# ten2net/Gym-Trading-Env

Hardware: AMD Instinct MI355X
Metric: env-steps/sec (higher is better)
Workload: dtype f64

## Files before the change

gym-trading-env_amd/csrc/gte_api.hip:

```cpp
#include <hip/hip_runtime.h>

#include <climits>
#include <cstdarg>
#include <cstdio>
#include <cstdlib>
#include <cstring>
#include <new>
#include <string>
#include <utility>
#include <vector>

#include "gte_launch.h"
#include "gte_ledger.h"
#include "gte_plan.h"

using gte::DatasetDesc;
using gte::EnvRec;
using gte::Params;
using gte_plan::LaunchPlan;
using gte_plan::SLIDE_AB_ORDER;
using gte_ledger::FLAGS;
using gte_ledger::WINDOW;
using gte_ledger::ledger;

// ... 380 lines not shown
  }
  double* d_pos = nullptr;
  chk(dev_alloc(E, &d_pos, GTE_MAX_POSITIONS));
  chk(dev_alloc(E, &E->d_ds, (size_t)p.D));
  if (rc == GTE_OK &&
      hipMemcpy(d_pos, cfg->positions, sizeof(double) * p.P, hipMemcpyHostToDevice) != hipSuccess)
    rc = fail(GTE_ERR_HIP, "copying positions failed");
  if (rc != GTE_OK) return create_failed(E, rc);
  p.positions = d_pos;
  p.ds = E->d_ds;
  E->owned.obs_elems_per_env = (int64_t)p.W * p.Fobs;
  p.final_obs = nullptr;
  p.obs = nullptr; p.reward = E->owned.reward; p.reward64 = E->owned.reward64;
  p.obs_rows = p.W; p.obs_head = 0; p.slide = 0;
  p.terminated = E->owned.terminated; p.truncated = E->owned.truncated;
  E->term_base = E->owned.term_count; p.term_ids = E->owned.term_ids;
  E->h_ds.assign((size_t)p.D, DatasetDesc{nullptr, nullptr, nullptr, nullptr, 0});
  for (auto& v : E->ds_allocs) v.assign((size_t)p.D, nullptr);

  rc = plan_launches(E);
  if (rc != GTE_OK) return create_failed(E, rc);
  if (hipDeviceSynchronize() != hipSuccess)
    return create_failed(E, fail(GTE_ERR_HIP, "hipDeviceSynchronize failed after allocation"));
  report_plan(E, "create");
  *out = E;
  return GTE_OK;
}

static int publish_signal_table(gte_env* E, int32_t d, const gte::SignalTable& t) {
  const gte::SignalTable before = E->h_sig[d];
  E->h_sig[d] = t;
  const hipError_t e = hipMemcpy(E->d_sig, E->h_sig.data(), sizeof(gte::SignalTable) * E->h_sig.size(),
                                 hipMemcpyHostToDevice);
  if (e != hipSuccess) {
    E->h_sig[d] = before;
    return fail(GTE_ERR_HIP, "publishing the signal table of dataset %d: %s", d, hipGetErrorString(e));
  }
  bool any = false;
  for (const gte::SignalTable& x : E->h_sig) any = any || x.base != nullptr;
  if (!any) E->sig_S = 0;
  return GTE_OK;
}

static int publish_period_row(gte_env* E, int32_t d, const gte::PeriodRow& r) {
  const gte::PeriodRow before = E->h_prow[d];
  E->h_prow[d] = r;
  const hipError_t e = hipMemcpy(E->d_prow, E->h_prow.data(), sizeof(gte::PeriodRow) * E->h_prow.size(),
                                 hipMemcpyHostToDevice);
  if (e != hipSuccess) {
    E->h_prow[d] = before;
    return fail(GTE_ERR_HIP, "publishing the period row of dataset %d: %s", d, hipGetErrorString(e));
  }
  if (before.base) (void)hipFree(const_cast<int8_t*>(before.base));
  if (E->pd_B > 0) E->pd_changed = true;
  return GTE_OK;
}

int gte_upload_dataset(gte_env* E, int32_t d, const float* feat, const double* close,
                       const double* high, const double* low, int64_t T) {
  if (!E) return fail(GTE_ERR_INVALID, "env is NULL");
  const Params& p = E->p;
  if (d < 0 || d >= p.D) return fail(GTE_ERR_INVALID, "dataset index %d out of range", d);
  if (!feat || !close) return fail(GTE_ERR_INVALID, "feat and close are required");
  if (T <= 0 || T > 0x7FFFFFF0ll) return fail(GTE_ERR_INVALID, "T out of range");
  const int64_t idx0 = p.has_window ? p.W - 1 : 0;
  if (T < idx0 + 2) return fail(GTE_ERR_INVALID, "dataset of %lld rows is too short for windows=%d",
                                (long long)T, p.W);
  if (p.max_dur > 0 && T - p.max_dur - idx0 <= idx0)
    return fail(GTE_ERR_INVALID, "low >= high: %lld rows cannot host episodes of %d steps",
                (long long)T, p.max_dur);
  if (E->finalized && p.persist && T > p.depth)
    return fail(GTE_ERR_STATE, "dyn_persist: cannot upload a longer dataset after the first reset");
  if (E->was_reset && T < E->h_ds[d].T)
    return fail(GTE_ERR_STATE, "dataset %d: cannot replace %lld rows by %lld after gte_reset "
                "(running environments may be past the new end); create a new env instead",
                d, (long long)E->h_ds[d].T, (long long)T);
  HIPCHK(hipSetDevice(E->cfg.device));
  HIPCHK(hipStreamSynchronize(E->stream));
  const void* srcs[4] = {feat, close, high, low};
  const size_t bytes[4] = {sizeof(float) * (size_t)T * p.Fobs, sizeof(double) * (size_t)T,
                           sizeof(double) * (size_t)T, sizeof(double) * (size_t)T};
  void* dev[4] = {nullptr, nullptr, nullptr, nullptr};
  auto undo = [&]() { for (void* q : dev) if (q) (void)hipFree(q); };
  for (int k = 0; k < 4; ++k) {
    if (!srcs[k]) continue;
    hipError_t e = hipMalloc(&dev[k], bytes[k]);
    if (e == hipSuccess && getenv("GTE_DEBUG_ALLOC"))
      fprintf(stderr, "[gte] dataset %d column %d at %p, %zu bytes\n", d, k, dev[k], bytes[k]);
    if (e == hipSuccess) e = hipMemcpy(dev[k], srcs[k], bytes[k], hipMemcpyHostToDevice);
    if (e != hipSuccess) {
      undo();
      return fail(e == hipErrorOutOfMemory ? GTE_ERR_OOM : GTE_ERR_HIP, "uploading dataset %d: %s", d,
                  hipGetErrorString(e));
    }
  }
  const DatasetDesc before = E->h_ds[d];
  E->h_ds[d] = DatasetDesc{(const float*)dev[0], (const double*)dev[1], (const double*)dev[2],
                           (const double*)dev[3], T};
  const hipError_t e = hipMemcpy(E->d_ds, E->h_ds.data(), sizeof(DatasetDesc) * p.D, hipMemcpyHostToDevice);
  if (e != hipSuccess) {
    E->h_ds[d] = before;
    undo();
    return fail(GTE_ERR_HIP, "publishing the descriptor of dataset %d: %s", d, hipGetErrorString(e));
  }
  for (int k = 0; k < 4; ++k) {
    if (E->ds_allocs[k][d]) (void)hipFree(E->ds_allocs[k][d]);
    E->ds_allocs[k][d] = dev[k];
  }
  if (E->d_sig && E->h_sig[d].base) TRY(publish_signal_table(E, d, gte::SignalTable{nullptr, 0}));
  if (E->d_prow && E->h_prow[d].base) TRY(publish_period_row(E, d, gte::PeriodRow{nullptr, 0}));
  return GTE_OK;
}

static int finalize(gte_env* E) {
  if (E->finalized) return GTE_OK;
  Params& p = E->p;
  int64_t maxT = 0;
  for (int d = 0; d < p.D; ++d) {
    if (E->h_ds[d].T <= 0) return fail(GTE_ERR_STATE, "dataset %d was never uploaded", d);
    if (E->h_ds[d].T > maxT) maxT = E->h_ds[d].T;
  }
  p.depth = p.persist ? maxT : p.W;
  size_t table_bytes = 0;
  for (int d = 0; d < p.D; ++d) table_bytes += (size_t)E->h_ds[d].T * p.Fobs * sizeof(float);
  gte_plan::affinity_after_upload(E->plan, plan_shape(E), table_bytes);
  TRY(dev_alloc(E, &p.ring, (size_t)p.N * p.depth * (p.nd ? p.nd : 1)));
  HIPCHK(hipDeviceSynchronize());
  report_plan(E, "finalize");
  E->finalized = true;
  return GTE_OK;
}

static int check_injection(const gte_env* E, size_t count, const int32_t* idx, const int32_t* pos,
                           const int32_t* ds) {
  const Params& p = E->p;
  int64_t maxT = 0, minT = INT64_MAX;
  for (int d = 0; d < p.D; ++d) {
    if (E->h_ds[d].T > maxT) maxT = E->h_ds[d].T;
    if (E->h_ds[d].T > 0 && E->h_ds[d].T < minT) minT = E->h_ds[d].T;
  }
  const int64_t idx0 = p.has_window ? p.W - 1 : 0;
  for (size_t i = 0; i < count; ++i) {
    if (pos && pos[i] >= p.P) return fail(GTE_ERR_INVALID, "injected position index %d >= %d", pos[i], p.P);
    if (ds && ds[i] >= p.D) return fail(GTE_ERR_INVALID, "injected dataset %d >= %d", ds[i], p.D);
    if (idx && idx[i] >= 0) {
      const int64_t T = (ds && ds[i] >= 0) ? E->h_ds[ds[i]].T : minT;
      if (idx[i] < idx0 || idx[i] > T - 2)
        return fail(GTE_ERR_INVALID, "injected start row %d outside [%lld, %lld]", idx[i],
                    (long long)idx0, (long long)(T - 2));
    }
  }
  return GTE_OK;
}

static int append_log(gte_env* E, const Params& p, const uint8_t* mask = nullptr) {
  if (E->cfg.log_steps <= 0) return GTE_OK;
  if (E->log_rows == 0) mask = nullptr;
  HIPCHK(gte::launch_log(p.rec, p.reward64, p.terminated, p.truncated, p.N, E->log_cursor + (E->term_slot ^ 1),
                         E->cfg.log_steps, E->log, mask, E->stream));
  if (!mask) E->log_rows += 1;
  return GTE_OK;
}

static int park_cursor(gte_env* E, int slot) {
  if (!E->log_cursor || E->term_slot == slot) return GTE_OK;
  HIPCHK(hipMemcpyAsync(E->log_cursor + slot, E->log_cursor + E->term_slot, sizeof(int64_t),
                        hipMemcpyDeviceToDevice, E->stream));
  return GTE_OK;
}

static int stage(gte_env* E, void* dst, const void* src, size_t bytes) {
  HIPCHK(hipMemcpyAsync(dst, src, bytes, hipMemcpyHostToDevice, E->stream));
  return GTE_OK;
}

static int ensure_owned_obs(gte_env* E) {
  Params& p = E->p;
  const size_t elems = (size_t)p.N * (size_t)p.W * (size_t)p.Fobs;
  bool fresh = false;
  if (!p.obs) {
    if (!E->owned.obs) { TRY(dev_alloc(E, &E->owned.obs, elems)); fresh = true; }
    p.obs = E->owned.obs;
  }
  if (E->cfg.final_obs && !p.final_obs) {
    if (!E->owned.final_obs) { TRY(dev_alloc(E, &E->owned.final_obs, elems)); fresh = true; }
    p.final_obs = E->owned.final_obs;
  }
  if (fresh) HIPCHK(hipDeviceSynchronize());
  return GTE_OK;
}

static int resort(gte_env* E) {
  E->steps_since_rebuild = 0;
  const hipError_t e = gte::launch_affinity_rebuild(E->p, E->d_bins, E->plan.n_bins_per_ds,
                                                    E->d_slot_of_rank, E->d_perm, E->stream);
  if (e != hipSuccess) {
    E->plan.affinity_period = 0;
    E->p.perm = nullptr;
    return fail(GTE_ERR_HIP, "re-sort of the processing order: %s", hipGetErrorString(e));
  }
  E->p.perm = E->d_perm;
  return GTE_OK;
}

int gte_reset(gte_env* E, const uint8_t* mask, const int32_t* inj_idx,
              const int32_t* inj_pos_index, const int32_t* inj_dataset) {
  if (!E) return fail(GTE_ERR_INVALID, "env is NULL");
  HIPCHK(hipSetDevice(E->cfg.device));
  TRY(ensure_owned_obs(E));
  TRY(finalize(E));
  TRY(check_injection(E, (size_t)E->p.N, inj_idx, inj_pos_index, inj_dataset));
  Params p = E->p;
  const bool fresh_run = E->sliding && !mask;
  if (fresh_run) p.obs_head = 0;
  ledger().wrote(E, {obs_span(E), flag_span(E, p.terminated), flag_span(E, p.truncated)}, false,
                 fresh_run ? FLAGS | WINDOW : FLAGS);
  const size_t N = (size_t)p.N;
  p.mask = nullptr; p.inj_idx = p.inj_pos = p.inj_ds = nullptr;
  if (mask) { TRY(stage(E, E->d_mask, mask, N)); p.mask = E->d_mask; }
  if (inj_idx) { TRY(stage(E, E->d_inj_idx, inj_idx, 4 * N)); p.inj_idx = E->d_inj_idx; }
  if (inj_pos_index) { TRY(stage(E, E->d_inj_pos, inj_pos_index, 4 * N)); p.inj_pos = E->d_inj_pos; }
  if (inj_dataset) { TRY(stage(E, E->d_inj_ds, inj_dataset, 4 * N)); p.inj_ds = E->d_inj_ds; }
  HIPCHK(hipMemsetAsync(E->term_base, 0, 2 * sizeof(int32_t), E->stream));
  TRY(park_cursor(E, 1));
  E->term_slot = 0;
  p.term_count = E->term_base;
  p.term_count_next = E->term_base + 1;
  const LaunchPlan& L = E->plan;
  HIPCHK(gte::launch_reset(p, L.vec, L.store, L.coop, L.stage, L.blocks, L.threads, E->stream));
  if (fresh_run) {
    E->p.obs_head = 0;
    ledger().establish(E, WINDOW, {obs_span(E)}, false);
  }
  TRY(append_log(E, p, p.mask));
  if (L.affinity_period > 0) TRY(resort(E));
  HIPCHK(hipStreamSynchronize(E->stream));
  E->was_reset = true;
  return GTE_OK;
}

int gte_set_autoreset_injection(gte_env* E, int32_t n, const int32_t* inj_idx,
                                const int32_t* inj_pos_index, const int32_t* inj_dataset) {
  if (!E) return fail(GTE_ERR_INVALID, "env is NULL");
  if (n < 0) return fail(GTE_ERR_INVALID, "n_episodes must be >= 0");
  for (int d = 0; d < E->p.D; ++d)
    if (E->h_ds[d].T <= 0) return fail(GTE_ERR_STATE, "upload every dataset before queueing draws");
  TRY(check_injection(E, (size_t)E->p.N * (size_t)n, inj_idx, inj_pos_index, inj_dataset));
  HIPCHK(hipSetDevice(E->cfg.device));
  HIPCHK(hipStreamSynchronize(E->stream));
  Params& p = E->p;
  const size_t count = (size_t)p.N * (size_t)n;
  auto put = [&](int32_t** slot, const int32_t* src, const int32_t** param) -> int {
    *param = nullptr;
    if (*slot) { (void)hipFree(*slot); *slot = nullptr; }
    if (!src || n == 0) return GTE_OK;
    void* dev = nullptr;
    HIPCHK(hipMalloc(&dev, sizeof(int32_t) * count));
    *slot = (int32_t*)dev;
    HIPCHK(hipMemcpy(dev, src, sizeof(int32_t) * count, hipMemcpyHostToDevice));
    *param = *slot;
    return GTE_OK;
  };
  TRY(put(&E->d_q_idx, inj_idx, &p.q_idx));
  TRY(put(&E->d_q_pos, inj_pos_index, &p.q_pos));
  TRY(put(&E->d_q_ds, inj_dataset, &p.q_ds));
  p.q_n = n;
  HIPCHK(gte::launch_rewind_queue(p.rec, p.N, E->stream));
  HIPCHK(hipStreamSynchronize(E->stream));
  HIPCHK(hipDeviceSynchronize());
  return GTE_OK;
}

static bool stream_capturing(gte_env* E) {
  hipStreamCaptureStatus capture = hipStreamCaptureStatusNone;
  if (hipStreamIsCapturing(E->stream, &capture) != hipSuccess) { (void)hipGetLastError(); capture = hipStreamCaptureStatusNone; }
  return capture == hipStreamCaptureStatusActive;
}

static void advance_term_slot(gte_env* E, Params& p) {
  E->term_slot ^= 1;
  p.term_count = E->term_base + E->term_slot;
  p.term_count_next = E->term_base + (E->term_slot ^ 1);
}

struct StepTargets {
  const int32_t* actions;
  float *obs, *reward;
  double* reward64;
  uint8_t *terminated, *truncated;
  bool own_obs;
};

static StepTargets own_targets(const gte_env* E, const int32_t* actions) {
  return {actions, E->p.obs, E->p.reward, E->p.reward64, E->p.terminated, E->p.truncated, true};
}

static int age_order(gte_env* E, int32_t steps) {
  if (E->plan.affinity_period > 0 && (E->steps_since_rebuild += steps) >= E->plan.affinity_period) {
    TRY(resort(E));
  }
  return GTE_OK;
}

static int enqueue_step(gte_env* E, const StepTargets& t, int store, bool capturing,
                        EnvRec* terminal_rec = nullptr) {
  const LaunchPlan& L = E->plan;
  const bool slides_own = t.own_obs && E->sliding;
  gte_ledger::Span obs = obs_span(E);
  const bool slide = slides_own && !capturing && ledger().holds(E, WINDOW, {obs}) && E->p.obs_head < L.slide_rows;
  const bool env_order = slide && !L.full_windows && !(L.slide_ab & SLIDE_AB_ORDER);
  if (env_order) { if (L.affinity_period > 0) E->steps_since_rebuild += 1; }
  else TRY(age_order(E, 1));
  Params p = E->p;
  if (env_order) p.perm = nullptr;
  if (terminal_rec) p.final_rec = terminal_rec;
  p.actions = t.actions; p.obs = t.obs; p.reward = t.reward; p.reward64 = t.reward64;
  p.terminated = t.terminated; p.truncated = t.truncated;
  if (!t.own_obs) {
    p.obs_rows = p.W; p.obs_head = 0;
    obs = {t.obs, sizeof(float) * (size_t)p.N * p.W * p.Fobs};
  } else if (E->sliding) {
    if (slide) {
      E->p.obs_head += 1;
      if (p.persist || p.final_obs)
        return fail(GTE_ERR_STATE, "internal: a sliding step with dyn_persist or final_obs (the planner grants neither)");
      p.slide = L.full_windows ? 0 : 1;
    } else {
      E->p.obs_head = 0;
    }
    p.obs_head = E->p.obs_head;
  }
  advance_term_slot(E, p);
  if (L.fused_log) {
    p.log = E->log;
    p.log_cursor = E->log_cursor + (E->term_slot ^ 1);
  }
  const gte_ledger::Span term = flag_span(E, p.terminated), trunc = flag_span(E, p.truncated);
  p.flags_sparse = !capturing && !L.always_dense && ledger().holds(E, FLAGS, {term, trunc}) ? 1 : 0;
  ledger().wrote(E, {obs, term, trunc}, capturing, FLAGS | WINDOW);
  const bool hot = L.hot_tu && gte::hot_tu_covers(p);
  if (p.slide) store = L.slide_store;
  if (hot && store == 2)
    HIPCHK(gte::launch_step_hot(p, L.blocks, L.threads, gte::lds_bytes(p, L.stage), E->stream));
  else if (hot && store == 1)
    HIPCHK(gte::launch_step_hot_nt(p, L.blocks, L.threads, gte::lds_bytes(p, L.stage), E->stream));
  else
    HIPCHK(gte::launch_step(p, L.vec, store, L.coop, L.stage, L.blocks, L.threads, E->stream));
  ledger().establish(E, FLAGS, {term, trunc}, capturing);
  if (slides_own) ledger().establish(E, WINDOW, {obs}, capturing);
  if (L.fused_log) E->log_rows += 1;
  else TRY(append_log(E, p));
  return GTE_OK;
}

int gte_step(gte_env* E, const int32_t* actions, int32_t actions_on_device) {
  if (!E) return fail(GTE_ERR_INVALID, "env is NULL");
  if (!E->was_reset) return fail(GTE_ERR_STATE, "gte_step before gte_reset");
  if (!actions) return fail(GTE_ERR_INVALID, "actions is NULL");
  const bool capturing = stream_capturing(E);
  if (capturing && !actions_on_device)
    return fail(GTE_ERR_STATE, "gte_step on a capturing stream needs device-resident actions "
                               "(a copy from pageable host memory cannot be captured)");
  if (!actions_on_device) {
    TRY(stage(E, E->d_actions, actions, sizeof(int32_t) * (size_t)E->p.N));
    actions = E->d_actions;
  }
  return enqueue_step(E, own_targets(E, actions), E->plan.store, capturing);
}

int gte_get_schedule(gte_env* E, gte_schedule* out) {
  if (!E || !out) return fail(GTE_ERR_INVALID, "NULL argument");
  out->log_rows = E->log_rows;
  out->term_slot = E->term_slot;
  out->steps_since_rebuild = E->steps_since_rebuild;
  return GTE_OK;
}

int gte_set_schedule(gte_env* E, const gte_schedule* s) {
  if (!E || !s) return fail(GTE_ERR_INVALID, "NULL argument");
  if ((s->term_slot != 0 && s->term_slot != 1) || s->log_rows < 0 || s->steps_since_rebuild < 0)
    return fail(GTE_ERR_INVALID, "not a schedule gte_get_schedule returned");
  E->log_rows = s->log_rows;
  E->term_slot = s->term_slot;
  E->steps_since_rebuild = s->steps_since_rebuild;
  ledger().withdraw(E, FLAGS | WINDOW);
  return GTE_OK;
}

int gte_advance_log(gte_env* E, int64_t rows) {
  if (!E) return fail(GTE_ERR_INVALID, "env is NULL");
  if (E->cfg.log_steps <= 0) return fail(GTE_ERR_STATE, "created with log_steps = 0");
  if (rows < 0) return fail(GTE_ERR_INVALID, "rows must be >= 0");
  E->log_rows += rows;
  return GTE_OK;
}

static void report_rollout_path(const char* path, int32_t n_steps) {
  if (debug_geometry()) fprintf(stderr, "[gte] rollout path: %s, %d steps\n", path, n_steps);
}

static int rollout(gte_env* E, const int32_t* actions, int32_t n_steps, const gte_rollout_bufs* b) {
  const size_t N = (size_t)E->p.N;
  const size_t V = (size_t)E->p.W * (size_t)E->p.Fobs;
  const LaunchPlan& L = E->plan;
  const int nt = (b->obs && E->cfg.nontemporal_obs == 3) ? 1 : L.store;
  const bool capturing = stream_capturing(E);
  const size_t rows = (size_t)n_steps * N;
  ledger().wrote(E, {{b->obs, sizeof(float) * rows * V}, {b->terminated, rows}, {b->truncated, rows},
                     flag_span(E, E->p.terminated), flag_span(E, E->p.truncated)}, capturing, WINDOW);
  auto step_row = [&](int32_t k) -> int {
    StepTargets t = own_targets(E, actions + (size_t)k * N);
    if (b->obs) { t.obs = b->obs + (size_t)k * N * V; t.own_obs = false; }
    if (b->reward) t.reward = b->reward + (size_t)k * N;
    if (b->reward64) t.reward64 = b->reward64 + (size_t)k * N;
    if (b->terminated) t.terminated = b->terminated + (size_t)k * N;
    if (b->truncated) t.truncated = b->truncated + (size_t)k * N;
    TRY(enqueue_step(E, t, nt, capturing));
    if (b->valuation) {
      hipError_t e = gte::launch_extract_state(E->p.rec, E->p.N, E->soa, E->stream);
      if (e == hipSuccess)
        e = hipMemcpyAsync(b->valuation + (size_t)k * N, E->soa.pv, 8 * N, hipMemcpyDeviceToDevice,
                           E->stream);
      if (e != hipSuccess) return fail(GTE_ERR_HIP, "rollout: %s", hipGetErrorString(e));
    }
    return GTE_OK;
  };
  if (!L.fused_rollout) {
    report_rollout_path("per-step", n_steps);
    for (int32_t k = 0; k < n_steps; ++k) TRY(step_row(k));
  } else if (!b->obs) {
    report_rollout_path(n_steps > 1 ? "state-only" : "per-step", n_steps);
    if (n_steps > 1) {
      TRY(age_order(E, n_steps - 1));
      gte::RolloutArgs r = {actions, n_steps - 1, nullptr, b->reward, b->reward64, b->terminated,
                            b->truncated, b->valuation, 0, 0, nullptr};
      Params ps = E->p;
      ps.perm = nullptr;
      const hipError_t le = gte::launch_rollout_state(ps, r, n_steps - 1, L.state_epw, E->stream);
      if (le != hipSuccess) return fail(GTE_ERR_HIP, "rollout launch: %s", hipGetErrorString(le));
    }
    TRY(step_row(n_steps - 1));
  } else {
    TRY(age_order(E, n_steps));
    Params p = E->p;
    if (L.resident_epb[nt] == 0) {
      DeviceChip chip(E);
      gte_plan::choose_resident_epb(E->plan, plan_shape(E), read_knobs(KNOBS_ROLLOUT), chip, nt);
      report_plan(E, "resident");
    }
    advance_term_slot(E, p);
    report_rollout_path(L.resident_epb[nt] > 0 ? "resident" : "gather", n_steps);
    if (L.resident_epb[nt] > 0) {
      p.perm = nullptr;
      if (!E->d_group_counter) TRY(dev_alloc_late(E, &E->d_group_counter, 4));
      HIPCHK(hipMemsetAsync(E->d_group_counter, 0, sizeof(int32_t), E->stream));
      const int epb = L.resident_epb[nt];
      const int n_groups = (p.N + epb - 1) / epb;
      gte::RolloutArgs r = {actions, n_steps, b->obs, b->reward, b->reward64, b->terminated,
                            b->truncated, b->valuation, epb, n_groups, E->d_group_counter};
      const int blocks = n_groups < L.resident_slots[nt] ? n_groups : L.resident_slots[nt];
      const hipError_t le = gte::launch_rollout_resident(p, r, nt, blocks, E->stream);
      if (le != hipSuccess) return fail(GTE_ERR_HIP, "rollout launch: %s", hipGetErrorString(le));
    } else {
      if (L.rollout_epw == 0) {
        DeviceChip chip(E);
        gte_plan::choose_rollout_epw(E->plan, plan_shape(E), chip, nt);
        report_plan(E, "gather");
      }
      p.epw = L.rollout_epw;
      const int r_blocks = gte::rollout_blocks(p.N, p.epw);
      gte::RolloutArgs r = {actions, n_steps, b->obs, b->reward, b->reward64, b->terminated,
                            b->truncated, b->valuation, 0, 0, nullptr};
      const hipError_t le = gte::launch_rollout(p, r, nt, r_blocks, E->stream);
      if (le != hipSuccess) return fail(GTE_ERR_HIP, "rollout launch: %s", hipGetErrorString(le));
    }
  }
  const size_t last = (size_t)(n_steps - 1) * N;
  if (b->reward) HIPCHK(hipMemcpyAsync(E->p.reward, b->reward + last, 4 * N, hipMemcpyDeviceToDevice, E->stream));
  if (b->reward64) HIPCHK(hipMemcpyAsync(E->p.reward64, b->reward64 + last, 8 * N, hipMemcpyDeviceToDevice, E->stream));
  if (b->terminated) HIPCHK(hipMemcpyAsync(E->p.terminated, b->terminated + last, N, hipMemcpyDeviceToDevice, E->stream));
  if (b->truncated) HIPCHK(hipMemcpyAsync(E->p.truncated, b->truncated + last, N, hipMemcpyDeviceToDevice, E->stream));
  return GTE_OK;
}

int gte_rollout(gte_env* E, const int32_t* actions, int32_t n_steps, const gte_rollout_bufs* b) {
  if (!E) return fail(GTE_ERR_INVALID, "env is NULL");
  if (!E->was_reset) return fail(GTE_ERR_STATE, "gte_rollout before gte_reset");
  if (!actions) return fail(GTE_ERR_INVALID, "actions is NULL");
  if (n_steps < 1) return fail(GTE_ERR_INVALID, "n_steps must be >= 1");
  static const gte_rollout_bufs none = {nullptr, nullptr, nullptr, nullptr, nullptr, nullptr};
  if (!b) b = &none;
  if (b->obs && ((uintptr_t)b->obs & 15)) return fail(GTE_ERR_INVALID, "obs must be 16-byte aligned");
  HIPCHK(hipSetDevice(E->cfg.device));
  const int rc = rollout(E, actions, n_steps, b);
  ledger().withdraw(E, FLAGS);
  return rc;
}

static hipError_t launch_lookup(gte_env* E, const int32_t* strategy, int32_t* actions) {
  if (E->exits.rules)
    return gte::launch_exit_actions(E->p, E->d_sig, E->sig_S, strategy, E->exits, actions, E->stream);
  return gte::launch_signal_actions(E->p, E->d_sig, E->sig_S, strategy, actions, E->stream);
}

static int backtest(gte_env* E, const int32_t* actions, const int32_t* strategy, int32_t n_steps, int32_t clear) {
  const size_t N = (size_t)E->p.N;
  const LaunchPlan& L = E->plan;
  const bool signals = actions == nullptr;
  ledger().wrote(E, {flag_span(E, E->p.terminated), flag_span(E, E->p.truncated)}, false, WINDOW);
  if (signals && !E->d_sig_actions) TRY(dev_alloc_late(E, &E->d_sig_actions, N));
  if (!E->bt_stats) {
    if (E->p.autoreset == GTE_AUTORESET_SAME_STEP && !E->p.final_rec) TRY(dev_alloc(E, &E->bt_final_rec, N));
    TRY(dev_alloc_late(E, &E->bt_stats, N));
    clear = 1;
  }
  if (E->tr_changed) clear = 1;
  E->tr_changed = false;
  gte_trade_stats* const trades = E->tr_on ? E->tr_stats : nullptr;
  if (E->pd_changed) clear = 1;
  E->pd_changed = false;
  const bool periods = E->pd_B > 0;
  const gte::Periods per = {E->d_prow, E->pd_stats, E->pd_B};
  EnvRec* const terminal = E->p.final_rec ? E->p.final_rec : E->bt_final_rec;
  Params ps = E->p;
  ps.perm = nullptr;
  ps.final_rec = terminal;
  hipError_t le = trades ? gte::launch_trade_begin(ps, E->bt_stats, trades, clear, E->stream)
                         : gte::launch_backtest_begin(ps, E->bt_stats, clear, E->stream);
  if (le != hipSuccess) return fail(GTE_ERR_HIP, "backtest launch: %s", hipGetErrorString(le));
  if (periods && clear)
    HIPCHK(hipMemsetAsync(E->pd_stats, 0, sizeof(gte_period_stats) * N * (size_t)E->pd_B, E->stream));
  auto step_and_fold = [&](int32_t k) -> int {
    if (signals) {
      const hipError_t se = launch_lookup(E, strategy, E->d_sig_actions);
      if (se != hipSuccess) return fail(GTE_ERR_HIP, "backtest launch: %s", hipGetErrorString(se));
    }
    const int32_t* const row = signals ? E->d_sig_actions : actions + (size_t)k * N;
    TRY(enqueue_step(E, own_targets(E, row), L.store, false, E->bt_final_rec));
    const hipError_t fe = trades    ? gte::launch_trade_fold(ps, E->bt_stats, trades, E->stream)
                          : periods ? gte::launch_period_fold(ps, E->bt_stats, per, E->stream)
                                    : gte::launch_backtest_fold(ps, E->bt_stats, E->stream);
    if (fe != hipSuccess) return fail(GTE_ERR_HIP, "backtest launch: %s", hipGetErrorString(fe));
    return GTE_OK;
  };
  if (!L.fused_rollout) {
    report_rollout_path(signals ? "backtest signals per-step" : "backtest per-step", n_steps);
    for (int32_t k = 0; k < n_steps; ++k) TRY(step_and_fold(k));
    return GTE_OK;
  }
  if (signals) report_rollout_path(n_steps > 1 ? "backtest signals summary" : "backtest signals per-step", n_steps);
  else report_rollout_path(n_steps > 1 ? "backtest summary" : "backtest per-step", n_steps);
  if (n_steps > 1) {
    TRY(age_order(E, n_steps - 1));
    const gte::SummarySource src = {actions, E->d_sig, E->sig_S, strategy, E->exits.rules ? &E->exits : nullptr};
    const int32_t k = n_steps - 1, epw = L.state_epw;
    le = trades    ? gte::launch_trade_summary(ps, src, E->bt_stats, trades, k, epw, E->stream)
         : periods ? gte::launch_period_summary(ps, src, E->bt_stats, per, k, epw, E->stream)
         : signals ? gte::launch_signal_summary(ps, src, E->bt_stats, k, epw, E->stream)
                   : gte::launch_backtest_summary(ps, src, E->bt_stats, k, epw, E->stream);
    if (le != hipSuccess) return fail(GTE_ERR_HIP, "backtest launch: %s", hipGetErrorString(le));
  }
  return step_and_fold(n_steps - 1);
}

static int backtest_entry(gte_env* E, const char* who, const int32_t* actions, const int32_t* strategy,
                          int32_t n_steps, int32_t clear, gte_backtest_stats** stats_device) {
  if (n_steps < 1) return fail(GTE_ERR_INVALID, "n_steps must be >= 1");
  if (stream_capturing(E))
    return fail(GTE_ERR_STATE, "%s inside a stream capture: a backtest is one launch already, run it eagerly", who);
  if (E->pd_B > 0)
    for (int d = 0; d < E->p.D; ++d)
      if (!E->d_prow || !E->h_prow[d].base)
        return fail(GTE_ERR_STATE, "%s: period tracking is on and dataset %d has no period row (gte_bind_periods)", who, d);
  HIPCHK(hipSetDevice(E->cfg.device));
  const int rc = backtest(E, actions, strategy, n_steps, clear);
  ledger().withdraw(E, FLAGS);
  if (stats_device) *stats_device = E->bt_stats;
  return rc;
}

int gte_backtest(gte_env* E, const int32_t* actions, int32_t n_steps, int32_t clear,
                 gte_backtest_stats** stats_device) {
  if (!E) return fail(GTE_ERR_INVALID, "env is NULL");
  if (!E->was_reset) return fail(GTE_ERR_STATE, "gte_backtest before gte_reset");
  if (!actions) return fail(GTE_ERR_INVALID, "actions is NULL");
  return backtest_entry(E, "gte_backtest", actions, nullptr, n_steps, clear, stats_device);
}

static int64_t round_up_16(int64_t T) { return (T + 15) / 16 * 16; }

static int builder_dataset(gte_env* E, const char* who, int32_t d, int64_t* T) {
  if (d < 0 || d >= E->p.D) return fail(GTE_ERR_INVALID, "dataset index %d out of range", d);
  if (stream_capturing(E)) return fail(GTE_ERR_STATE, "%s inside a stream capture", who);
  *T = E->h_ds[d].T;
  if (*T <= 0) return fail(GTE_ERR_STATE, "%s: dataset %d was never uploaded", who, d);
  return GTE_OK;
}

static int check_stride(const char* name, int64_t stride, size_t elem, int64_t T, int32_t d) {
  const int64_t k = 16 / (int64_t)elem;
  if (stride % k == 0 && stride >= round_up_16(T)) return GTE_OK;
  return fail(GTE_ERR_INVALID, "%s %lld%s: a multiple of %lld and >= %lld (the %lld rows of dataset %d rounded up "
              "to 16) required", name, (long long)stride, elem == sizeof(float) ? " floats" : "", (long long)k,
              (long long)round_up_16(T), (long long)T, d);
}

struct RowSpan { const void* base; int64_t rows, stride; size_t elem; };
static bool spans_overlap(const RowSpan& r, const RowSpan& w, int64_t T16) {
  const uintptr_t r0 = (uintptr_t)r.base, w0 = (uintptr_t)w.base;
  const uintptr_t r1 = r0 + r.elem * (size_t)((r.rows - 1) * r.stride + T16);
  const uintptr_t w1 = w0 + w.elem * (size_t)((w.rows - 1) * w.stride + T16);
  return r0 < w1 && w0 < r1;
}

static int check_strategies(const gte_env* E, int32_t n_strategies) {
  if (!E) return fail(GTE_ERR_INVALID, "env is NULL");
  if (n_strategies < 1) return fail(GTE_ERR_INVALID, "n_strategies must be >= 1");
  return GTE_OK;
}

static int check_n_periods(int32_t n_periods, int lo) {
  if (n_periods >= lo && n_periods <= GTE_MAX_PERIODS) return GTE_OK;
  return fail(GTE_ERR_INVALID, "n_periods %d outside [%d, %d]", n_periods, lo, GTE_MAX_PERIODS);
}

static int check_period_mask(const uint64_t* period_mask) {
  return period_mask ? GTE_OK : fail(GTE_ERR_INVALID, "period_mask is NULL");
}

static int check_reduce_args(gte_env* E, const char* who, const void* records, const int32_t* group_offsets,
                             const int32_t* group_envs, const void* out) {
  if (!out || ((uintptr_t)out & 15)) return fail(GTE_ERR_INVALID, "out_device must be a 16-byte aligned device array");
  if ((uintptr_t)records & 15) return fail(GTE_ERR_INVALID, "records must be 16-byte aligned");
  if ((group_offsets == nullptr) != (group_envs == nullptr))
    return fail(GTE_ERR_INVALID, "group_offsets and group_envs: both or neither");
  if (((uintptr_t)group_offsets & 3) || ((uintptr_t)group_envs & 3))
    return fail(GTE_ERR_INVALID, "the group lists must be 4-byte aligned");
  if (stream_capturing(E)) return fail(GTE_ERR_STATE, "%s inside a stream capture", who);
  return GTE_OK;
}

static int check_rank_args(gte_env* E, const char* who, int32_t k, int32_t metric, int lo, int hi, const void* stats,
                           const int32_t* top_index, const double* top_score, const double* scores) {
  if (k < 1 || k > GTE_RANK_MAX) return fail(GTE_ERR_INVALID, "k must lie in [1, %d]", GTE_RANK_MAX);
  if (metric < lo || metric > hi) return fail(GTE_ERR_INVALID, "metric %d unknown", metric);
// ... 1023 lines not shown
```

gym-trading-env_amd/csrc/gte_launch.h:

```cpp
#pragma once
#include "gte_device.h"

namespace gte {

using gte_plan::LEAN_MAX_ROWS;
using gte_plan::RES_LDS_MAX;
using gte_plan::RES_NEW;
using gte_plan::RES_OWNERS;
using gte_plan::ROLLOUT_WAVES;
inline int rollout_blocks(int n_envs, int epw) {
  return (int)((((int64_t)n_envs + epw - 1) / epw + ROLLOUT_WAVES - 1) / ROLLOUT_WAVES);
}
constexpr size_t LDS_OPT_IN = 64 * 1024;

inline uint64_t magic40(uint32_t d) { return ((1ull << 40) + d - 1) / d; }

hipError_t launch_step(const Params& p, int vec, int nt, bool coop, int stage, int blocks, int threads,
                       hipStream_t stream);
hipError_t launch_reset(const Params& p, int vec, int nt, bool coop, int stage, int blocks, int threads,
                        hipStream_t stream);
size_t lds_bytes(const Params& p, int stage);
size_t lds_image_bytes(int epw, int W, int nd, bool final_obs, bool log_row, int stage);
hipError_t launch_add_orders(const Params& p, const int32_t* pos_index, const double* limit,
                             const uint8_t* persistent, hipStream_t stream);
hipError_t launch_affinity_rebuild(const Params& p, int32_t* bins, int n_bins_per_ds, const int32_t* slot_of_rank,
                                   int32_t* perm_out, hipStream_t stream);
struct StateSoA {
  int32_t *idx, *step, *pos, *dsi, *start, *episode, *needs_reset;
  double *asset, *fiat, *ia, *ifi, *pv, *realpos;
};
hipError_t launch_extract_state(const EnvRec* rec, int n, const StateSoA& o, hipStream_t stream);
hipError_t launch_rewind_queue(EnvRec* rec, int n, hipStream_t stream);

hipError_t launch_step_hot(const Params& p, int blocks, int threads, size_t smem, hipStream_t stream);
hipError_t launch_step_hot_nt(const Params& p, int blocks, int threads, size_t smem, hipStream_t stream);
int hot_blocks_per_cu(size_t smem);
int hot_blocks_per_cu_nt(size_t smem);

struct RolloutArgs {
  const int32_t* actions;
  int32_t K;
  float* obs;
  float* reward;
  double* reward64;
  uint8_t *terminated, *truncated;
  double* valuation;
  int32_t epb;
  int32_t n_groups;
  int32_t* group_counter;
};
size_t resident_lds_bytes(const Params& p, int epb);
int resident_blocks_per_cu(const Params& p, int epb, int nt);
hipError_t launch_rollout_resident(const Params& p, const RolloutArgs& r, int nt, int blocks, hipStream_t stream);
hipError_t launch_rollout_state(const Params& p, const RolloutArgs& r, int n_steps, int epw, hipStream_t stream);
int rollout_blocks_per_cu(const Params& p, int nt);
hipError_t launch_rollout(const Params& p, const RolloutArgs& r, int nt, int blocks, hipStream_t stream);

struct SignalTable {
  const int8_t* base;
  int64_t stride;
};
struct ExitRules {
  const gte_exit_rule* rules;
  const int32_t* rule_of_env;
  gte_exit_state* state;
  int32_t n_rules;
};
struct SummarySource {
  const int32_t* actions;
  const SignalTable* tables;
  int32_t S;
  const int32_t* strategy;
  const ExitRules* rules;
};
struct PeriodRow {
  const int8_t* base;
  int32_t len;
};
struct Periods {
  const PeriodRow* rows;
  gte_period_stats* records;
  int32_t B;
};
inline bool tables_usable(const SignalTable* tables, int S) { return tables && S >= 1; }
inline bool exit_rules_usable(const ExitRules& r) { return r.rules && r.n_rules >= 1 && r.state; }
inline bool summary_refused(const Params& p, const SummarySource& src, int epw) {
  return p.log.rows != nullptr || (p.autoreset == GTE_AUTORESET_SAME_STEP && p.final_rec == nullptr) || epw < 1 ||
         epw > 64 ||
         (!src.actions && (!tables_usable(src.tables, src.S) || (src.rules && !exit_rules_usable(*src.rules))));
}
inline bool fold_refused(const Params& p) { return p.autoreset == GTE_AUTORESET_SAME_STEP && p.final_rec == nullptr; }

hipError_t launch_backtest_begin(const Params& p, gte_backtest_stats* stats, int clear, hipStream_t stream);
hipError_t launch_backtest_summary(const Params& p, const SummarySource& src, gte_backtest_stats* stats, int n_steps,
                                   int epw, hipStream_t stream);
hipError_t launch_signal_summary(const Params& p, const SummarySource& src, gte_backtest_stats* stats, int n_steps,
                                 int epw, hipStream_t stream);
hipError_t launch_backtest_fold(const Params& p, gte_backtest_stats* stats, hipStream_t stream);
hipError_t launch_signal_actions(const Params& p, const SignalTable* tables, int S, const int32_t* strategy,
                                 int32_t* actions, hipStream_t stream);

hipError_t launch_exit_init(gte_exit_state* state, int n, hipStream_t stream);
hipError_t launch_exit_actions(const Params& p, const SignalTable* tables, int S, const int32_t* strategy,
                               const ExitRules& rules, int32_t* actions, hipStream_t stream);
hipError_t launch_exit_summary(const Params& p, const SummarySource& src, gte_backtest_stats* stats, int n_steps,
                               int epw, hipStream_t stream);

hipError_t launch_trade_begin(const Params& p, gte_backtest_stats* stats, gte_trade_stats* trades, int clear,
                              hipStream_t stream);
hipError_t launch_trade_summary(const Params& p, const SummarySource& src, gte_backtest_stats* stats,
                                gte_trade_stats* trades, int n_steps, int epw, hipStream_t stream);
hipError_t launch_trade_fold(const Params& p, gte_backtest_stats* stats, gte_trade_stats* trades,
                             hipStream_t stream);

hipError_t launch_period_summary(const Params& p, const SummarySource& src, gte_backtest_stats* stats,
                                 const Periods& per, int n_steps, int epw, hipStream_t stream);
hipError_t launch_period_fold(const Params& p, gte_backtest_stats* stats, const Periods& per, hipStream_t stream);

hipError_t launch_build_signals(const float* indicators, int n_indicators, int64_t ind_stride,
                                const gte_signal_rule* rules, int n_rules, int64_t T, int8_t* table,
                                int64_t row_stride, hipStream_t stream);

hipError_t launch_compose_signals(const int8_t* clauses, int n_clause_rows, int64_t clause_stride,
                                  const gte_signal_compose* specs, int n_specs, int64_t T, int8_t* table,
                                  int64_t row_stride, hipStream_t stream);

hipError_t launch_build_indicators(const DatasetDesc& ds, int Fobs, int n_static, const gte_indicator_spec* specs,
                                   int n_specs, const float* input, int n_inputs, int64_t input_stride, float* bank,
                                   int64_t ind_stride, hipStream_t stream);

hipError_t launch_reduce_strategies(const gte_backtest_stats* records, int n_envs, int n_strategies,
                                    int64_t env_id_base, const int32_t* group_offsets, const int32_t* group_envs,
                                    gte_strategy_stats* out, hipStream_t stream);
int64_t rank_scratch_entries(int n_strategies, int which);
hipError_t launch_rank_strategies(const gte_strategy_stats* stats, int n_strategies, int metric, int64_t min_episodes,
                                  int k, int32_t* top_index, double* top_score, double* scores, double* const* cand_score,
                                  int32_t* const* cand_index, hipStream_t stream);
hipError_t launch_rank_select(int n_strategies, int k, int32_t* top_index, double* top_score, double* const* cand_score,
                              int32_t* const* cand_index, hipStream_t stream);

hipError_t launch_reduce_trade_stats(const gte_trade_stats* records, int n_envs, int n_strategies, int64_t env_id_base,
                                     const int32_t* group_offsets, const int32_t* group_envs,
                                     gte_strategy_trade_stats* out, hipStream_t stream);
hipError_t launch_trade_scores(const gte_strategy_trade_stats* stats, int n_strategies, int metric, int64_t min_trades,
                               double* scores, double* cand_score, int32_t* cand_index, hipStream_t stream);

hipError_t launch_reduce_period_stats(const gte_period_stats* records, int n_envs, int n_periods, int n_strategies,
                                      int64_t env_id_base, const int32_t* group_offsets, const int32_t* group_envs,
                                      gte_strategy_period_stats* out, hipStream_t stream);
hipError_t launch_period_scores(const gte_strategy_period_stats* stats, int n_strategies, int n_periods,
                                const uint64_t period_mask[2], int metric, int64_t min_steps, double* scores,
                                double* cand_score, int32_t* cand_index, hipStream_t stream);

hipError_t launch_bootstrap_weights(int n, int n_resamples, uint32_t thr, int always, uint64_t seed, double* weights,
                                    hipStream_t stream);
size_t reality_check_scratch_bytes(int n_strategies, int n, int n_resamples);
hipError_t launch_reality_check(const gte_strategy_period_stats* stats, int n_strategies, int n_periods,
                                const uint64_t period_mask[2], int n, const double* benchmark, const double* weights,
                                int n_resamples, const gte_reality_check_out& out, void* scratch,
                                hipStream_t stream);

hipError_t launch_log(const EnvRec* rec, const double* reward64, const uint8_t* term, const uint8_t* trunc, int n,
                      const int64_t* cursor, int L, const LogArrays& o, const uint8_t* mask, hipStream_t stream);
hipError_t launch_set_log_reward(LogRow* rows, const int64_t* last, int L, int n, const double* reward,
                                 hipStream_t stream);
hipError_t launch_set_dynamic(const Params& p, const float* values, uint32_t mask, hipStream_t stream);
hipError_t launch_set_dynamic_columns(const Params& p, const void* const* cols, const int32_t* is_f64,
                                      hipStream_t stream);
hipError_t launch_apply_reward(const Params& p, const double* reward, LogRow* rows, const int64_t* last,
                               int terminal_view, hipStream_t stream);
struct LogPack {
  int32_t* n_rows;
  int32_t *idx, *step, *pos, *dsi;
  double *pv, *realpos, *reward, *asset, *fiat, *ia, *ifi;
  uint8_t* flags;
};
hipError_t launch_pack_log(const LogArrays& log, int N, int L, long long rows_written, const int32_t* ids,
                           int n_ids, int max_rows, int finished, int frozen_runs, const EnvRec* final_rec,
                           const double* reward64, const LogPack& o, hipStream_t stream);
hipError_t launch_snapshot(const EnvRec* rec, const double* reward64, const uint8_t* term, const uint8_t* trunc,
                           const float* obs, int64_t obs_elems, int64_t obs_stride, int first, int count, void* dst,
                           float* dst_obs, hipStream_t stream);

const char* rccl_load();
const char* rccl_error(int code);
int rccl_unique_id(uint8_t* out128);
int rccl_comm_init(void** comm, const uint8_t* id128, int rank, int world);
int rccl_allgather_bytes(void* comm, const void* src, void* dst, size_t bytes, hipStream_t stream);
int rccl_comm_destroy(void* comm);

}
```

gym-trading-env_amd/csrc/gte_plan.h:

```cpp
#pragma once
#include <cstddef>
#include <cstdint>
#include <cstdio>

#include "../../include/gte.h"

#ifndef GTE_WAVES
#define GTE_WAVES 4
#endif
#ifndef GTE_LEAN_U
#define GTE_LEAN_U 4
#endif

namespace gte_plan {

constexpr int LEAN_MAX_ROWS = 512;
constexpr int ROLLOUT_WAVES = 4;
constexpr int RES_NEW = 2;
constexpr int RES_OWNERS = 192;
constexpr size_t RES_LDS_MAX = 160 * 1024;

enum { SLIDE_AB_ORDER = 1, SLIDE_AB_STORE = 2 };

struct LaunchPlan {
  int vec = 1, blocks = 0, threads = 256;
  bool coop = false;
  int stage = 0;
  int hot_per_cu = 0;
  int store = 0;
  int slide_store = 0;
  bool hot_tu = false;
  bool fused_log = false;
  bool always_dense = false;
  int slide_rows = 0;
  bool full_windows = false;
  int slide_ab = 0;
  bool fused_rollout = false;
  bool resident_rollout = false;
  int affinity_period = 0;
  int n_bins_per_ds = 0;
  int state_epw = 0;
  int rollout_epw = 0;
  int resident_slots[3] = {0, 0, 0};
  int resident_epb[3] = {0, 0, 0};
  int epw = 0;
  int lean_rows = 0;
  int hot_lds = 0;
  int debug = 0;
};

struct Shape {
  int N = 0, D = 0, W = 1;
  bool has_window = false;
  int Fobs = 0, nd = 0;
  bool persist = false;
  int max_dur = 0;
  bool final_obs = false;
  int log_steps = 0;
  int envs_per_wave = 0, nontemporal_obs = 0, obs_slack_rows = 0, affinity_period = 0, kernel_variant = 0,
      debug_flags = 0;
};

struct Knobs {
  bool slide_full_windows = false;
  int slide_ab = 0;
  int slide_store = -1;
  bool has_affinity_bins = false;
  int affinity_bins = 0;
  bool has_resident_epb = false;
  int resident_epb = 0;
  bool debug_geometry = false;
};

struct Chip {
  int n_cu = 0;
  virtual size_t step_lds_bytes(int epw, int stage) = 0;
  virtual int hot_per_cu(int store, size_t smem) = 0;
  virtual size_t resident_lds_bytes(int epb) = 0;
  virtual int resident_per_cu(int epb, int store) = 0;
  virtual int gather_per_cu(int epw, int store) = 0;
  virtual ~Chip() = default;
};

inline void step_geometry(LaunchPlan& L, const Shape& p, const Knobs& k, Chip& chip, bool hot_ok, bool lean_ok) {
  L.vec = (p.Fobs % 4 == 0) ? 4 : 1;
  const int64_t vpe = (int64_t)p.W * p.Fobs / L.vec;
  int epw = p.envs_per_wave;
  if (epw == 0) {
    epw = (vpe >= 64) ? 16 : 64;
    while (epw > 1 && ((int64_t)p.N + epw - 1) / epw < 4096) epw >>= 1;
    while (epw < 64 && (int64_t)epw * vpe < 64) epw <<= 1;
    const bool residency_shape = L.vec == 4 && vpe >= 64 && p.nd > 0 && !p.persist && !p.final_obs &&
                                 (L.store == 1 || L.store == 2) && hot_ok;
    if (residency_shape) {
      const int64_t n_cu = chip.n_cu;
      int some_per_cu = 0;
      int64_t fewest = 0;
      int one_round_epw = 0, one_round_per_cu = 0;
      for (int e = 64 / GTE_WAVES; e >= 1; --e) {
        if ((int64_t)e * vpe < 64) break;
        const size_t smem = chip.step_lds_bytes(e, 1);
        const int per_cu = chip.hot_per_cu(L.store, smem);
        if (per_cu <= 0) break;
        if (e <= 8 || !some_per_cu) some_per_cu = per_cu;
        const int64_t wgs = ((int64_t)p.N + GTE_WAVES * e - 1) / (GTE_WAVES * e);
        const int64_t busiest = (wgs + n_cu - 1) / n_cu;
        if (k.debug_geometry)
          fprintf(stderr, "[gte] envs/wave %2d: LDS %5zu B, %d workgroups/CU resident, %lld workgroups, "
                          "%lld on the busiest CU\n", e, smem, per_cu, (long long)wgs, (long long)busiest);
        if (busiest <= per_cu && busiest * GTE_WAVES >= 16 && (fewest == 0 || busiest * e < fewest)) {
          fewest = busiest * e;
          one_round_epw = e;
          one_round_per_cu = per_cu;
        }
      }
      if (one_round_epw) {
        epw = one_round_epw;
        L.hot_per_cu = one_round_per_cu;
      } else if (some_per_cu) {
        L.hot_per_cu = some_per_cu;
        const int64_t target = (int64_t)p.N >= 120000 ? 640 : 960;
        int e = (int)((target + vpe / 2) / vpe);
        e = e < 1 ? 1 : (e > 64 / GTE_WAVES ? 64 / GTE_WAVES : e);
        while (e < 64 / GTE_WAVES && (int64_t)e * vpe < 64) ++e;
        epw = e;
        if (lean_ok) {
          int lean_e = 0;
          for (int c = 1; c <= 64 / GTE_WAVES; ++c)
            if (((int64_t)c * vpe) % (64 * GTE_LEAN_U) == 0 && (int64_t)c * p.W <= LEAN_MAX_ROWS) { lean_e = c; break; }
          if (lean_e) {
            int c = lean_e;
            while (c * 2 <= 64 / GTE_WAVES && (int64_t)c * vpe < 1280 && (int64_t)c * 2 * p.W <= LEAN_MAX_ROWS) c *= 2;
            if ((int64_t)p.N >= 200000 && c * 2 <= 64 / GTE_WAVES && (int64_t)c * 2 * p.W <= LEAN_MAX_ROWS) c *= 2;
            epw = c;
          }
        }
      }
    }
  }
  while (epw > 1 && (int64_t)epw * vpe > (1 << 20)) epw >>= 1;
  while (epw > 1 && (int64_t)epw * GTE_WAVES * p.W * (p.nd ? p.nd : 1) * 4 > 32 * 1024) epw >>= 1;
  L.epw = epw;
  const int64_t waves = ((int64_t)p.N + epw - 1) / epw;
  L.threads = 64 * GTE_WAVES;
  L.blocks = (int)((waves + GTE_WAVES - 1) / GTE_WAVES);
}

inline void plan_affinity(LaunchPlan& L, const Shape& p, const Knobs& k) {
  int auto_period = 128;
  if (p.max_dur > 0) {
    auto_period = p.max_dur / 16;
    auto_period = auto_period < 8 ? 8 : (auto_period > 128 ? 128 : auto_period);
  }
  const int period = p.affinity_period == 0 ? auto_period : p.affinity_period;
  const int EPB = L.epw * GTE_WAVES;
  const int n_wg = (p.N + EPB - 1) / EPB;
  if (!(period > 0 && n_wg >= 64 && (int64_t)p.W * p.Fobs * 4 >= 512)) return;
  int nb = 8192 / p.D;
  if (k.has_affinity_bins) nb = k.affinity_bins / p.D;
  nb = nb < 1 ? 1 : (nb > 4096 ? 4096 : nb);
  L.n_bins_per_ds = nb;
  L.affinity_period = period;
}

inline void fill_slot_of_rank(const Shape& p, int epw, int32_t* slot_of_rank) {
  const int64_t EPB = (int64_t)epw * GTE_WAVES;
  const int64_t n_wg = (p.N + EPB - 1) / EPB;
  for (int x = 0; x < 8; ++x)
    for (int64_t b = x; b < n_wg; b += 8)
      for (int64_t sl = b * EPB; sl < (b + 1) * EPB && sl < p.N; ++sl) *slot_of_rank++ = (int32_t)sl;
}

inline int slide_store_policy(const LaunchPlan& L, const Shape& p, const Knobs& k, Chip& chip) {
  if (L.slide_rows == 0 || L.full_windows || (L.slide_ab & SLIDE_AB_STORE)) return L.store;
  int s = p.nontemporal_obs;
  if (s == 3) s = ((size_t)p.N * (p.W + L.slide_rows) * p.Fobs * sizeof(float) > ((size_t)190 << 20)) ? 1 : L.store;
  if (s != L.store && L.hot_tu && s != 0) {
    const size_t smem = chip.step_lds_bytes(L.epw, L.stage);
    const int per_cu = chip.hot_per_cu(s, smem);
    if (per_cu < (L.blocks + chip.n_cu - 1) / chip.n_cu) s = L.store;
  }
  if (k.slide_store >= 0) s = k.slide_store;
  return s;
}

inline LaunchPlan plan_create(const Shape& p, const Knobs& k, Chip& chip) {
  LaunchPlan L;
  const int kv = p.kernel_variant;
  L.store = p.nontemporal_obs;
  if (L.store == 3) L.store = ((size_t)p.N * p.W * p.Fobs * sizeof(float) > ((size_t)190 << 20)) ? 1 : 2;
  step_geometry(L, p, k, chip, !(kv & (GTE_KV_PER_WAVE_PHASE_A | GTE_KV_NO_LDS_STAGING)), !(kv & GTE_KV_GENERIC_COPY));
  L.debug = p.debug_flags;
  L.coop = (L.epw * GTE_WAVES <= 64) && !(kv & GTE_KV_PER_WAVE_PHASE_A);
  L.stage = (p.nd > 0 && chip.step_lds_bytes(L.epw, 1) <= 48 * 1024 && !(kv & GTE_KV_NO_LDS_STAGING)) ? (p.persist ? 2 : 1) : 0;
  L.lean_rows = (L.vec == 4 && L.stage == 1 && !(kv & GTE_KV_GENERIC_COPY)) ? 1 : 0;
  L.hot_lds = (kv & GTE_KV_RECORD_DIRECT) ? 0 : 1;
  const bool hot_launch_shape = L.vec == 4 && L.coop && L.stage == 1;
  L.hot_tu = hot_launch_shape && !(kv & GTE_KV_SHARED_TU);
  L.fused_log = p.log_steps > 0 && !(kv & GTE_KV_LOG_SEPARATE);
  L.always_dense = (kv & GTE_KV_DENSE_FLAGS) != 0;
  L.slide_rows = 0;
  if (hot_launch_shape && (int64_t)p.W * p.Fobs / 4 >= 64 && p.has_window && !p.persist && !p.final_obs &&
      p.log_steps == 0 && p.obs_slack_rows >= 0)
    L.slide_rows = p.obs_slack_rows > 0 ? p.obs_slack_rows : 2 * p.W / 5;
  L.full_windows = k.slide_full_windows;
  L.slide_ab = k.slide_ab;
  L.slide_store = slide_store_policy(L, p, k, chip);
  L.fused_rollout = hot_launch_shape && !p.final_obs && p.log_steps == 0 && !(kv & GTE_KV_ROLLOUT_PER_STEP);
  L.resident_rollout = p.W >= 2 && !(kv & GTE_KV_ROLLOUT_GATHER);
  L.state_epw = (p.N >= 64 * 1024) ? 64 : 32;
  plan_affinity(L, p, k);
  return L;
}

inline void affinity_after_upload(LaunchPlan& L, const Shape& p, uint64_t table_bytes) {
  if (L.affinity_period > 0 && p.affinity_period == 0 && table_bytes > ((uint64_t)64 << 20)) L.affinity_period = 0;
}

inline void choose_resident_epb(LaunchPlan& L, const Shape& p, const Knobs& k, Chip& chip, int nt) {
  L.resident_epb[nt] = -1;
  const int64_t FV = p.Fobs / 4;
  if (!L.resident_rollout) return;
  const int n_cu = chip.n_cu;
  double best = 0.0;
  for (int e = 64; e >= 1; --e) {
    if (k.has_resident_epb && k.resident_epb != e) continue;
    if ((int64_t)e * FV > RES_NEW * RES_OWNERS) continue;
    const size_t smem = chip.resident_lds_bytes(e);
    if (smem > RES_LDS_MAX) continue;
    const int per_cu = chip.resident_per_cu(e, nt);
    if (per_cu <= 0) continue;
    const int64_t slots = (int64_t)per_cu * n_cu;
    const int64_t wgs = ((int64_t)p.N + e - 1) / e;
    const double rounds = wgs > slots ? (double)wgs / (double)slots : 1.0;
    const double live = (double)(wgs < slots ? (wgs + n_cu - 1) / n_cu : per_cu);
    const double us_bw = live * e * (double)p.W * p.Fobs * 4.0 / 22.0e3;
    static const double kAlone[5] = {1.7, 1.7, 1.10, 1.05, 1.0};
    const double alone = kAlone[per_cu < 4 ? per_cu : 4];
    const double cost = rounds * (us_bw > 3.0 ? us_bw : 3.0) * alone;
    if (k.debug_geometry)
      fprintf(stderr, "[gte] resident rollout, %2d envs/workgroup: LDS %6zu B, %d workgroups/CU, "
                      "%lld groups, %.2f round(s), cost %.1f\n", e, smem, per_cu, (long long)wgs, rounds, cost);
    if (best == 0.0 || cost < best * 0.999) {
      best = cost;
      L.resident_epb[nt] = e;
      L.resident_slots[nt] = (int)slots;
    }
  }
}

inline void choose_rollout_epw(LaunchPlan& L, const Shape& p, Chip& chip, int nt) {
  L.rollout_epw = L.epw;
  if (p.envs_per_wave != 0) return;
  for (int e = 1; e <= 16; ++e) {
    if ((int64_t)e * p.W * p.Fobs / 4 < 64) continue;
    const int per_cu = chip.gather_per_cu(e, nt);
    const int64_t wgs = ((int64_t)p.N + ROLLOUT_WAVES * e - 1) / (ROLLOUT_WAVES * e);
    if (per_cu > 0 && wgs <= (int64_t)per_cu * chip.n_cu) { L.rollout_epw = e; break; }
    if (e == 16) L.rollout_epw = 16;
  }
}

inline void print_plan(FILE* out, const char* when, const LaunchPlan& L) {
  fprintf(out, "[gte] plan: when=%s vec=%d blocks=%d threads=%d coop=%d stage=%d hot_per_cu=%d store=%d slide_store=%d "
          "hot_tu=%d fused_log=%d always_dense=%d slide_rows=%d full_windows=%d slide_ab=%d fused_rollout=%d "
          "resident_rollout=%d affinity_period=%d n_bins_per_ds=%d state_epw=%d rollout_epw=%d resident_slots=%d,%d,%d "
          "resident_epb=%d,%d,%d epw=%d lean_rows=%d hot_lds=%d debug=%d\n", when, L.vec, L.blocks, L.threads,
          (int)L.coop, L.stage, L.hot_per_cu, L.store, L.slide_store, (int)L.hot_tu, (int)L.fused_log, (int)L.always_dense,
          L.slide_rows, (int)L.full_windows, L.slide_ab, (int)L.fused_rollout, (int)L.resident_rollout, L.affinity_period,
          L.n_bins_per_ds, L.state_epw, L.rollout_epw, L.resident_slots[0], L.resident_slots[1], L.resident_slots[2],
          L.resident_epb[0], L.resident_epb[1], L.resident_epb[2], L.epw, L.lean_rows, L.hot_lds, L.debug);
}

}
```

Measured before the change: 3.847 billion.

## Add single-wave slide step kernel for large env counts

Adds a dedicated one-wave-per-block kernel for the sliding-window step path. It is used when the env count is large and the env-order path is active. Each wave handles 32 (or 64) envs, runs phase A, then copies only the newest obs row with the dyn-feature tail patched in; envs that need a full window fall back to a phase_b gather. The aim is to cut the per-block overhead and cross-wave synchronisation of the four-wave hot kernel for the slide step. In exchange it adds another code path with its own LDS layout and new A/B flags.

```diff
diff --git a/gym-trading-env_amd/csrc/gte_api.hip b/gym-trading-env_amd/csrc/gte_api.hip
--- a/gym-trading-env_amd/csrc/gte_api.hip
+++ b/gym-trading-env_amd/csrc/gte_api.hip
@@ -706,6 +706,12 @@
   return GTE_OK;
 }
 
+static void report_step_path(const char* path, int epw, int blocks) {
+  if (!debug_geometry()) return;
+  if (epw > 0) fprintf(stderr, "[gte] step path: %s epw=%d blocks=%d\n", path, epw, blocks);
+  else fprintf(stderr, "[gte] step path: %s\n", path);
+}
+
 static int enqueue_step(gte_env* E, const StepTargets& t, int store, bool capturing,
                         EnvRec* terminal_rec = nullptr) {
   const LaunchPlan& L = E->plan;
@@ -744,7 +750,15 @@
   ledger().wrote(E, {obs, term, trunc}, capturing, FLAGS | WINDOW);
   const bool hot = L.hot_tu && gte::hot_tu_covers(p);
   if (p.slide) store = L.slide_store;
-  if (hot && store == 2)
+  int wave_epw = 0;
+  const int wave_blocks =
+      (p.slide && !p.perm && hot && !p.debug) ? gte_plan::slide_wave_geometry(L, plan_shape(E), &wave_epw) : 0;
+  report_step_path(wave_blocks > 0 ? "slide-wave" : (p.slide ? "slide" : "full"), wave_epw, wave_blocks);
+  if (wave_blocks > 0) {
+    Params pw = p;
+    pw.epw = wave_epw;
+    HIPCHK(gte::launch_step_slide(pw, store, wave_blocks, E->stream));
+  } else if (hot && store == 2)
     HIPCHK(gte::launch_step_hot(p, L.blocks, L.threads, gte::lds_bytes(p, L.stage), E->stream));
   else if (hot && store == 1)
     HIPCHK(gte::launch_step_hot_nt(p, L.blocks, L.threads, gte::lds_bytes(p, L.stage), E->stream));
diff --git a/gym-trading-env_amd/csrc/gte_launch.h b/gym-trading-env_amd/csrc/gte_launch.h
--- a/gym-trading-env_amd/csrc/gte_launch.h
+++ b/gym-trading-env_amd/csrc/gte_launch.h
@@ -36,6 +36,8 @@
 hipError_t launch_step_hot_nt(const Params& p, int blocks, int threads, size_t smem, hipStream_t stream);
 int hot_blocks_per_cu(size_t smem);
 int hot_blocks_per_cu_nt(size_t smem);
+
+hipError_t launch_step_slide(const Params& p, int nt, int blocks, hipStream_t stream);
 
 struct RolloutArgs {
   const int32_t* actions;
diff --git a/gym-trading-env_amd/csrc/gte_plan.h b/gym-trading-env_amd/csrc/gte_plan.h
--- a/gym-trading-env_amd/csrc/gte_plan.h
+++ b/gym-trading-env_amd/csrc/gte_plan.h
@@ -20,7 +20,8 @@
 constexpr int RES_OWNERS = 192;
 constexpr size_t RES_LDS_MAX = 160 * 1024;
 
-enum { SLIDE_AB_ORDER = 1, SLIDE_AB_STORE = 2 };
+enum { SLIDE_AB_ORDER = 1, SLIDE_AB_STORE = 2, SLIDE_AB_FOUR_WAVES = 4, SLIDE_AB_WAVE_EPW = 8, SLIDE_AB_WAVE_ANY_SIZE = 16 };
+constexpr int SLIDE_WAVE_MIN_ENVS = 49152;
 
 struct LaunchPlan {
   int vec = 1, blocks = 0, threads = 256;
@@ -184,6 +185,16 @@
   return s;
 }
 
+inline int slide_wave_geometry(const LaunchPlan& L, const Shape& p, int* epw) {
+  *epw = 0;
+  if (!L.hot_tu || L.slide_rows == 0 || L.full_windows || (L.slide_ab & SLIDE_AB_FOUR_WAVES) || p.N <= 0) return 0;
+  if (p.N < SLIDE_WAVE_MIN_ENVS && !(L.slide_ab & SLIDE_AB_WAVE_ANY_SIZE)) return 0;
+  if ((int64_t)64 * p.W * p.Fobs / 4 > (1 << 20)) return 0;
+  const int e = (L.slide_ab & SLIDE_AB_WAVE_EPW) ? 64 : 32;
+  *epw = e;
+  return (int)(((int64_t)p.N + e - 1) / e);
+}
+
 inline LaunchPlan plan_create(const Shape& p, const Knobs& k, Chip& chip) {
   LaunchPlan L;
   const int kv = p.kernel_variant;
diff --git a/gym-trading-env_amd/csrc/gte_slide.hip b/gym-trading-env_amd/csrc/gte_slide.hip
--- /dev/null
+++ b/gym-trading-env_amd/csrc/gte_slide.hip
@@ -0,0 +1,113 @@
+#define GTE_HOT_ONLY 1
+#include "gte_step.h"
+
+namespace gte {
+
+constexpr int SLIDE_LDS_BYTES = 64 * (16 + 64 + 4 * GTE_MAX_DYN + 4);
+
+#ifndef GTE_SLIDE_U
+#define GTE_SLIDE_U 8
+#endif
+
+template <int NT, int U, typename Between>
+__device__ inline void slide_rows(const Params& p, const WgLds& L, int n_env, int lane, uint64_t fv_magic,
+                                  Between between) {
+  const uint32_t FV = (uint32_t)p.Fobs / 4u;
+  const uint32_t total = (uint32_t)n_env * FV;
+  const int64_t row = (int64_t)(p.W - 1) * FV;
+  float4_t* const obs0 = (float4_t*)obs_window0(p) + row;
+  const int64_t ES4 = obs_env_stride(p) / 4;
+  for (uint32_t k0 = 0u; k0 < total; k0 += 64u * U) {
+    float4_t v[U];
+    uint32_t rr[U];
+    int32_t env[U], sl[U];
+    bool ok[U];
+#pragma unroll
+    for (int u = 0; u < U; ++u) {
+      const uint32_t k = k0 + (uint32_t)u * 64u + (uint32_t)lane;
+      ok[u] = k < total;
+      const uint32_t kk = ok[u] ? k : 0u;
+      const uint32_t el = fastdiv40(kk, fv_magic);
+      rr[u] = kk - el * FV;
+      sl[u] = (int)el;
+      const JobRec j = L.job[sl[u]];
+      env[u] = j.env;
+      ok[u] = ok[u] && (j.meta & (uint32_t)JOB_SLIDES);
+      if constexpr (NT == 2) v[u] = float4_t{0.0f, 0.0f, 0.0f, 0.0f};
+      if (ok[u]) v[u] = load_global<float4_t>(j.src, row + (int64_t)rr[u]);
+    }
+    if (k0 == 0u) between();
+    if constexpr (NT == 2) {
+#pragma unroll
+      for (int u = 0; u < U; ++u) asm volatile("" : "+v"(v[u]));
+    }
+#pragma unroll
+    for (int u = 0; u < U; ++u) {
+      if (!ok[u]) continue;
+      if (rr[u] == FV - 1u) {
+        float x[GTE_MAX_DYN];
+#pragma unroll
+        for (int i = 0; i < GTE_MAX_DYN; ++i) x[i] = L.cur[sl[u] * GTE_MAX_DYN + i];
+        set_tail(v[u], p.nd, x);
+      }
+      store_out<NT>(obs0 + (int64_t)env[u] * ES4 + (int64_t)rr[u], v[u]);
+    }
+  }
+}
+
+template <int NT>
+__global__ __launch_bounds__(64) void gte_slide_kernel(const Params p, const uint64_t vpe_magic,
+                                                       const uint64_t fv_magic) {
+  [[maybe_unused]] constexpr int MODE = MODE_STEP;
+  __shared__ __attribute__((aligned(16))) unsigned char smem[SLIDE_LDS_BYTES];
+  const int lane = threadIdx.x;
+  if (blockIdx.x == 0 && lane == 0) p.term_count_next[0] = 0;
+  const int first = blockIdx.x * p.epw;
+  if (first >= p.N) return;
+  const int n_env = min(p.epw, p.N - first);
+  GTE_STAMP(0);
+  const WgLds L = carve_lds(smem, 64, false, false);
+  const bool active = lane < n_env;
+  L.job[lane].env = active ? first + lane : -1;
+  GTE_STAMP(1);
+
+  ObsJob job;
+  const lds_byte_ptr hot = p.hot_lds ? (lds_byte_ptr)(L.hot + 64 * lane) : (lds_byte_ptr) nullptr;
+  phase_a<MODE_STEP>(p, active ? first + lane : 0, active, lane, job, nullptr, true, nullptr, nullptr, nullptr, true,
+                     nullptr, nullptr, hot);
+  publish_job(L, lane, job);
+  __builtin_amdgcn_fence(__ATOMIC_RELEASE, "wavefront");
+  __builtin_amdgcn_wave_barrier();
+  __builtin_amdgcn_fence(__ATOMIC_ACQUIRE, "wavefront");
+  GTE_STAMP(6);
+
+  slide_rows<NT, GTE_SLIDE_U>(p, L, n_env, lane, fv_magic, [&] {
+    if (p.hot_lds) flush_hot_records(p, L, 0, n_env, lane);
+  });
+  const uint32_t m = L.job[lane].meta;
+  unsigned long long full = __ballot(active && (m & 1u) && !(m & (uint32_t)JOB_SLIDES));
+  const uint32_t VPE = (uint32_t)(p.W * p.Fobs) / 4u;
+  while (full) {
+    const uint32_t el = (uint32_t)(__ffsll((long long)full) - 1);
+    full &= full - 1ull;
+    phase_b<4, NT, STAGE_NONE, GTE_GATHER_U>(p, L, 0, n_env, lane, vpe_magic, fv_magic, el * VPE, (el + 1u) * VPE);
+  }
+  GTE_STAMP(7);
+}
+
+hipError_t launch_step_slide(const Params& p, int nt, int blocks, hipStream_t stream) {
+  if (!hot_tu_covers(p)) return hipErrorInvalidValue;
+  if (!p.slide || p.perm || p.persist || p.final_obs || p.debug || p.Fobs % 4 != 0 || p.epw < 1 || p.epw > 64 ||
+      (int64_t)blocks * p.epw < p.N)
+    return hipErrorInvalidValue;
+  const uint64_t vm = magic40((uint32_t)(p.W * p.Fobs) / 4), fm = magic40((uint32_t)p.Fobs / 4);
+  switch (nt) {
+    case 0: hipLaunchKernelGGL(gte_slide_kernel<0>, dim3(blocks), dim3(64), 0, stream, p, vm, fm); break;
+    case 1: hipLaunchKernelGGL(gte_slide_kernel<1>, dim3(blocks), dim3(64), 0, stream, p, vm, fm); break;
+    case 2: hipLaunchKernelGGL(gte_slide_kernel<2>, dim3(blocks), dim3(64), 0, stream, p, vm, fm); break;
+    default: return hipErrorInvalidValue;
+  }
+  return hipGetLastError();
+}
+
+}
```

New measurement: 3.930 billion, median of 5. 1.02x the previous value.
